# quantumjot/sequitr

Hardware: AMD Instinct MI355X
Metric: segmented Mpixels/sec on 512x512 tiles; IoU vs reference (higher is better)
Workload: dtype f32; 1 GPU; U-Net 2-class inference, launches of 32 512x512x1 tiles, fp32 (BASELINE.json configs[1]: filters 16-32-64-128-256, eltwise_mul bridge); logits + uint8 argmax mask; one 32-tile batch per GPU per step; tiles_this_rank=32

## Files before the change

### include/sequitr_hip.h

```cpp
#ifndef SEQUITR_HIP_H
#define SEQUITR_HIP_H

#include <stdint.h>

#ifdef __cplusplus
extern "C" {
#endif

#define SQ_OK 0
#define SQ_EINVAL (-1)
#define SQ_ELAUNCH (-2)
#define SQ_EALIGN (-3)

#define SQ_ACT_NONE 0
#define SQ_ACT_RELU 1
#define SQ_ACT_LEAKY 2

#define SQ_BRIDGE_NONE 0
#define SQ_BRIDGE_ADD 1
#define SQ_BRIDGE_MUL 2
#define SQ_BRIDGE_SUB 3

int sq_version(void);
const char *sq_last_error(void);
// ... 126 lines not shown
int sq_wgan_losses_fwd_f32(const float *Dz, const float *Dx, const float *gn2, float *out2, int N, void *stream);
int sq_wgan_losses_bwd_f32(const float *Dz, const float *Dx, const float *gn2, const float *g_dloss, const float *g_gloss,
                           float *dDz, float *dDx, float *dgn2, int N, void *stream);

int sq_mosaic_pack_f32(const float *x, float *m, int N, int H, int W, int C, int R, int Cc, void *stream);
int sq_mosaic_unpack_f32(const float *m, float *y, int N, int H, int W, int C, int R, int Cc, void *stream);

int64_t sq_dense_workspace_f32(int M, int K, int N);
int sq_dense_fwd_f32(const float *x, const float *w, const float *bias, float *y, float *workspace, int M, int K, int N,
                     float wscale, int act, void *stream);
int sq_dense_wgrad_f32(const float *x, const float *dy, float *dw, float *db, int M, int K, int N, float scale, int accumulate,
                       void *stream);

int64_t sq_wgrad1x1_small_workspace_f32(int64_t npix, int Ca, int Cb);
int sq_wgrad1x1_small_f32(const float *a, const float *b, float *m, float *workspace, int64_t npix, int Ca, int Cb,
                          void *stream);


int sq_conv2d_concat_nhwc_fwd_f32(const float *xa, const float *xb, const float *w, const float *bias, float *y, int N,
                                  int H, int W, int Ca, int Cout, int K, int act, void *stream);

int sq_conv3x3_pool_fwd_f32(const float *x, const float *w, const float *bias, float *y, float *pooled,
                            int N, int H, int W, int Cin, int Cout, int act, void *stream);

int sq_conv3x3_head_fwd_f32(const float *x, const float *w, const float *bias, const float *head_w,
                            const float *head_b, float *logits, uint8_t *mask, int N, int H, int W,
                            int Cin, int head_c, int act, void *stream);

int sq_conv3x3_first_block_fwd_f32(const float *x, const float *w1, const float *b1, const float *w2,
                                   const float *b2, float *y, float *pooled, int N, int H, int W,
                                   void *stream);

int sq_convT_conv3x3_fwd_f32(const float *x_low, const float *wt, const float *bt, const float *skip, int bridge,
                             const float *w, const float *bias, float *y, int N, int H, int W, int act, void *stream);


int64_t sq_conv_packed_weights_elems_bf16(int K, int Cin, int Cout);
int sq_conv_pack_weights_bf16(const float *w, void *wp, int K, int Cin, int Cout, float wscale, int transform,
                              void *stream);
int sq_conv_pack_weights_multi_bf16(const float *base, void *out, const int32_t *table, int n_entries,
                                    int total_items, void *stream);
int sq_conv_pack_weights_multi_scaled_bf16(const float *base, void *out, const int32_t *table, const float *scales,
                                           int n_entries, int total_items, void *stream);

int sq_conv2d_nhwc_fwd_bf16(const void *x, const void *wp, const float *bias, void *y, int N, int H, int W,
                            int Cin, int Cout, int K, int act, void *stream);
// ... 423 lines not shown
```

### sequitr_amd/_lib.py

```python
import ctypes
import os

_HERE = os.path.dirname(os.path.abspath(__file__))
LIB_PATH = os.path.join(_HERE, "_build", "libsequitr_hip.so")

c_void_p, c_int, c_float, c_int64 = ctypes.c_void_p, ctypes.c_int, ctypes.c_float, ctypes.c_int64


class WgradItem(ctypes.Structure):
    _fields_ = [("x", c_void_p), ("dy", c_void_p), ("dw", c_void_p), ("db", c_void_p),
                ("N", ctypes.c_int32), ("H", ctypes.c_int32), ("W", ctypes.c_int32), ("Cin", ctypes.c_int32),
                ("Cout", ctypes.c_int32), ("K", ctypes.c_int32), ("convT_cout", ctypes.c_int32), ("dw_scale", c_float),
                ("accumulate", ctypes.c_int32), ("mosaic_R", ctypes.c_int32), ("mosaic_Cc", ctypes.c_int32),
                ("reserved", ctypes.c_int32)]

SIGNATURES = {
    "sq_version": (c_int, []),
    "sq_last_error": (ctypes.c_char_p, []),
    "sq_conv2d_nhwc_fwd_f32": (c_int, [c_void_p] * 4 + [c_int] * 6 + [c_float, c_int, c_void_p]),
    "sq_maxpool2x2_fwd_f32": (c_int, [c_void_p] * 2 + [c_int] * 4 + [c_void_p]),
    "sq_avgpool2x2_fwd_f32": (c_int, [c_void_p] * 2 + [c_int] * 4 + [c_void_p]),
    "sq_convT2x2s2_nhwc_fwd_f32": (c_int, [c_void_p] * 5 + [c_int] * 6 + [c_void_p]),
    "sq_bridge_fwd_f32": (c_int, [c_void_p] * 3 + [c_int64, c_int, c_void_p]),
    "sq_conv1x1_argmax_fwd_f32": (c_int, [c_void_p] * 5 + [c_int] * 5 + [c_void_p]),
# ... 127 lines not shown
    "sq_broadcast2x2_act_bwd_f32": (c_int, [c_void_p] * 3 + [c_int] * 4 + [c_float, c_int, c_void_p]),
    "sq_resize_nearest_f32": (c_int, [c_void_p] * 2 + [c_int] * 6 + [c_void_p]),
    "sq_lerp_f32": (c_int, [c_void_p] * 3 + [c_int64, c_int64, c_float, c_void_p, c_void_p]),
    "sq_scale_f32": (c_int, [c_void_p] * 2 + [c_int64, c_int64, c_float, c_void_p, c_int, c_void_p]),
    "sq_act_fwd_f32": (c_int, [c_void_p] * 2 + [c_int64, c_int, c_void_p]),
    "sq_dot_per_sample_workspace_f32": (c_int64, [c_int]),
    "sq_dot_per_sample_f32": (c_int, [c_void_p] * 4 + [c_int, c_int64, c_void_p]),
    "sq_mbstd_fwd_f32": (c_int, [c_void_p] * 3 + [c_int, c_int64, c_void_p]),
    "sq_mbstd_map_workspace": (c_int64, [c_int]),
    "sq_mbstd_map_fwd_f32": (c_int, [c_void_p] * 3 + [c_int, c_int, c_int64, c_int, c_void_p]),
    "sq_mbstd_map_bwd_f32": (c_int, [c_void_p] * 4 + [c_int, c_int, c_int64, c_int, c_void_p]),
    "sq_mbstd_map_bwd2_f32": (c_int, [c_void_p] * 6 + [c_int, c_int, c_int64, c_int, c_void_p]),
    "sq_mbstd_map_fwd_bf16": (c_int, [c_void_p] * 3 + [c_int, c_int, c_int64, c_int, c_void_p]),
    "sq_mbstd_map_bwd_bf16": (c_int, [c_void_p] * 4 + [c_int, c_int, c_int64, c_int, c_void_p]),
    "sq_mbstd_map_bwd2_bf16": (c_int, [c_void_p] * 6 + [c_int, c_int, c_int64, c_int, c_void_p]),
    "sq_wgan_losses_fwd_f32": (c_int, [c_void_p] * 4 + [c_int, c_void_p]),
    "sq_wgan_losses_bwd_f32": (c_int, [c_void_p] * 8 + [c_int, c_void_p]),
    "sq_dense_wgrad_f32": (c_int, [c_void_p] * 4 + [c_int] * 3 + [c_float, c_int, c_void_p]),
    "sq_wgrad1x1_small_workspace_f32": (c_int64, [c_int64, c_int, c_int]),
    "sq_wgrad1x1_small_f32": (c_int, [c_void_p] * 4 + [c_int64, c_int, c_int, c_void_p]),
    "sq_conv2d_concat_nhwc_fwd_f32": (c_int, [c_void_p] * 5 + [c_int] * 7 + [c_void_p]),
    "sq_conv3x3_pool_fwd_f32": (c_int, [c_void_p] * 5 + [c_int] * 6 + [c_void_p]),
    "sq_conv3x3_head_fwd_f32": (c_int, [c_void_p] * 7 + [c_int] * 6 + [c_void_p]),
    "sq_conv3x3_first_block_fwd_f32": (c_int, [c_void_p] * 7 + [c_int] * 3 + [c_void_p]),
    "sq_conv_packed_weights_elems_bf16": (c_int64, [c_int] * 3),
    "sq_conv_pack_weights_bf16": (c_int, [c_void_p] * 2 + [c_int] * 3 + [c_float, c_int, c_void_p]),
    "sq_conv2d_nhwc_fwd_bf16": (c_int, [c_void_p] * 4 + [c_int] * 7 + [c_void_p]),
    "sq_conv2d_nhwc_fwd_mixed_f32": (c_int, [c_void_p] * 4 + [c_int] * 7 + [c_void_p]),
    "sq_conv2d_nhwc_wgrad_workspace_mixed_f32": (c_int64, [c_int] * 6),
    "sq_conv2d_nhwc_wgrad_mixed_f32": (c_int, [c_void_p] * 5 + [c_int] * 6 + [c_void_p]),
    "sq_conv2d_nhwc_wgrad_scaled_mixed_f32": (c_int, [c_void_p] * 5 + [c_int] * 6 + [c_float, c_void_p]),
    "sq_conv2d_nhwc_wgrad_scaled_f32": (c_int, [c_void_p] * 5 + [c_int] * 6 + [c_float, c_void_p]),
    "sq_conv3x3_first_fwd_bf16": (c_int, [c_void_p] * 4 + [c_int] * 6 + [c_void_p]),
    "sq_conv2d_nhwc_wgrad_workspace_bf16": (c_int64, [c_int] * 6),
    "sq_conv2d_nhwc_wgrad_bf16": (c_int, [c_void_p] * 5 + [c_int] * 6 + [c_void_p]),
    "sq_convT2x2s2_wgrad_bf16": (c_int, [c_void_p] * 5 + [c_int] * 5 + [c_void_p]),
    "sq_cast_f32_to_bf16": (c_int, [c_void_p] * 2 + [c_int64, c_void_p]),
    "sq_cast_bf16_to_f32": (c_int, [c_void_p] * 2 + [c_int64, c_void_p]),
    "sq_head_concat_fwd_bf16": (c_int, [c_void_p] * 3 + [c_int64, c_int, c_void_p]),
    "sq_head_concat_bwd_bf16": (c_int, [c_void_p] * 3 + [c_int64, c_int, c_void_p]),
    "sq_maxpool2x2_fwd_bf16": (c_int, [c_void_p] * 2 + [c_int] * 4 + [c_void_p]),
    "sq_maxpool2x2_bwd_bf16": (c_int, [c_void_p] * 3 + [c_int] * 4 + [c_void_p]),
    "sq_conv_pack_weights_multi_bf16": (c_int, [c_void_p, c_void_p, c_void_p, c_int, c_int, c_void_p]),
    "sq_conv_pack_weights_multi_scaled_bf16": (c_int, [c_void_p] * 4 + [c_int, c_int, c_void_p]),
    "sq_conv2d_nhwc_fwd_dropout_bf16": (c_int, [c_void_p] * 4 + [c_int] * 7 + [c_float, ctypes.c_uint32, c_void_p, c_void_p]),
    "sq_conv3x3_first_fwd_mask_bf16": (c_int, [c_void_p] * 5 + [c_int] * 6 + [c_void_p]),
# ... 99 lines not shown
```

### sequitr_amd/networks/unet.py

```python
import contextlib
import logging

import numpy as np
import torch

from .. import functional as F
from .. import functional_bf16 as FB
from .. import ops

DEFAULT_FILTERS = (16, 32, 64, 128, 256)
DEFAULT_DROPOUT = 0.4
BRIDGE_TYPES = ('eltwise_add', 'eltwise_mul', 'eltwise_sub', 'concat', None)

TRAIN, EVAL, PREDICT = 'train', 'eval', 'infer'

logger = logging.getLogger('worker_process')


def variance_scaling(shape, rng, scale=1.0):
    fan_in = float(shape[-2] * int(np.prod(shape[:-2])))
    std = np.sqrt(scale / max(1.0, fan_in)) / .87962566103423978
    out = rng.standard_normal(size=shape)
    bad = np.abs(out) > 2.0
    while bad.any():
# ... 191 lines not shown
        dev = params.get('device', None)
        self.device = torch.device(dev) if dev is not None else torch.device('cuda', torch.cuda.current_device())
        if self.device.type != 'cuda':
            raise RuntimeError('UNet2D runs on the HIP back end only (device=%s)' % self.device)
        if tuple(self.kernel) not in ((3, 3), (1, 1)):
            raise ValueError('kernel %s unsupported: the HIP conv kernels are 3x3 or 1x1' % (self.kernel,))
        self._params = dict(params)
        self._seed = params.get('seed', 0)
        self._rng = np.random.default_rng(self._seed)
        self._vars = {}
        self._loaded, self._creatable = False, set()
        self._dropout_calls = 0
        self._builds = 0
        self.dropout_masks = None
        self.fuse = bool(params.get('fuse', True))
        self.fuse_up = bool(params.get('fuse_up', True))
        self.up_kernel = tuple(params.get('up_kernel', (2, 2)))
        if self.up_kernel not in ((2, 2), (3, 3)):
            raise ValueError('up_kernel %s unsupported: (2,2) or (3,3)' % (self.up_kernel,))
        self.batch_norm = bool(params.get('batch_norm', False))
        self.bn_eps = float(params.get('bn_epsilon', ops.BN_EPS))
        self.bn_momentum = float(params.get('bn_momentum', ops.BN_MOMENTUM))
        self._mask = None

    @classmethod
    def variable_shapes(cls, params):
        return unet_variable_shapes(params)

    def get_variable(self, name, shape, init):
        key = self.scope + '/' + name
        v = self._vars.get(key)
        if v is None:
            if self._loaded and key not in self._creatable:
                raise KeyError('variable %s is not in the loaded model (load_state_dict(strict=False) to allow '
                               'missing variables to be initialised)' % key)
            v = torch.from_numpy(init(shape)).to(self.device)
            self._vars[key] = v
        elif tuple(v.shape) != tuple(shape):
            raise ValueError('variable %s has shape %s, wanted %s' % (key, tuple(v.shape), tuple(shape)))
        return v

    def _kernel(self, shape):
        return self.get_variable('kernel', shape, lambda s: variance_scaling(s, self._rng))

    def _bias(self, n):
        return self.get_variable('bias', (n,), lambda s: np.zeros(s, np.float32))
# ... 5 lines not shown
        req = dict(unet_variable_shapes(self._params))
        opt = {}
        if self.batch_norm:
            for k, shp in list(req.items()):
                if k.endswith('/gamma'):
                    sc = k.rsplit('/', 1)[0]
                    opt[sc + '/moving_mean'] = opt[sc + '/moving_variance'] = shp
        return req, opt

    def load_state_dict(self, weights, strict=True):
        req, opt = self.expected_variables()
        if strict:
            missing = [k for k in req if k not in weights]
            unexpected = [k for k in weights if k not in req and k not in opt]
            bad = [(k, tuple(np.shape(weights[k])), tuple(s)) for k, s in list(req.items()) + list(opt.items())
                   if k in weights and tuple(np.shape(weights[k])) != tuple(s)]
            if missing or unexpected or bad:
                raise ValueError('load_state_dict: model does not fit this %s configuration -- missing %s; unexpected %s; '
                                 'shape mismatches (key, got, wanted) %s' % (self.__class__.__name__, missing[:6],
                                                                             unexpected[:6], bad[:6]))
            self._loaded, self._creatable = True, set(opt)
        for k, v in weights.items():
            self._vars[k] = torch.as_tensor(np.ascontiguousarray(v, dtype=np.float32)).to(self.device)

    def initialize(self):
        self.load_state_dict(self._initial_weights(), strict=False)
        return self

    def _initial_weights(self):
        return init_unet_weights(self._params, self._seed)

    def reshape_input(self, features):
        if isinstance(features, np.ndarray):
            features = torch.from_numpy(np.require(features, np.float32, ['C', 'W']))
        if not isinstance(features, torch.Tensor):
            raise TypeError('features must be a numpy array or a torch tensor')
        features = features.to(self.device, dtype=torch.float32, non_blocking=True)
        return UNet.reshape_input(self, features).contiguous()

    def conv_layer(self, x, filters):
        k = tuple(self.kernel)
        w, b = self._kernel(k + (x.shape[-1], filters)), self._bias(filters)
        if self.batch_norm:
            z = F.conv2d(x, w, b, act=None) if self.training else ops.conv2d(x, w, b, act=None)
            return self.batch_norm_layer(z, act='relu')
        if self.training:
            return F.conv2d(x, w, b, act='relu')
        return ops.conv2d(x, w, b, act='relu')

    def batch_norm_layer(self, z, act=None):
        n = z.shape[-1]
        gamma = self.get_variable('gamma', (n,), lambda s: np.ones(s, np.float32))
        beta = self.get_variable('beta', (n,), lambda s: np.zeros(s, np.float32))
        mmean = self.get_variable('moving_mean', (n,), lambda s: np.zeros(s, np.float32))
        mvar = self.get_variable('moving_variance', (n,), lambda s: np.ones(s, np.float32))
        if self.training:
            return F.batch_norm_train(z, gamma, beta, mmean, mvar, self.bn_eps, self.bn_momentum, act=act)
        return ops.bn_inference(z, gamma, beta, mmean, mvar, self.bn_eps, act=act)

    def conv_layer_1x1(self, x, filters):
        w, b = self._kernel((1, 1, x.shape[-1], filters)), self._bias(filters)
        small = filters <= 7 and x.shape[-1] % 4 == 0
        if self.training:
            if small and filters <= 4 and x.shape[-1] in (8, 16, 32):
                return F.conv1x1_head(x, w, b)
            return F.conv2d(x, w, b, act=None)
        if small:
            logits, self._mask = ops.conv1x1_argmax(x, w, b)
            return logits
        return ops.conv2d(x, w, b, act=None)

# ... 77 lines not shown
    def _v(self, path, kind, shape):
        scopes = path.split('/')
        self._scopes.extend(scopes)
        try:
            return self._kernel(shape) if kind == 'kernel' else self._bias(shape[0])
        finally:
            del self._scopes[-len(scopes):]

    def _build_fused(self, features):
        f = list(self.filters)
        L = len(f)
        x = self.reshape_input(features)
        net, pooled = [], None
        for i in range(L):
            s = 'UNet/down%d' % i
            cin = x.shape[-1] if i == 0 else f[i - 1]
            w1, b1 = self._v(s + '/conv1', 'kernel', (3, 3, cin, f[i])), self._v(s + '/conv1', 'bias', (f[i],))
            w2, b2 = self._v(s + '/conv2', 'kernel', (3, 3, f[i], f[i])), self._v(s + '/conv2', 'bias', (f[i],))
            src = x if i == 0 else pooled
            last = i == L - 1
            if i == 0 and cin == 1 and f[0] == 16:
                y, pooled = ops.conv3x3_first_block(src, w1, b1, w2, b2, want_pool=not last)
            else:
                c1 = ops.conv2d(src, w1, b1, act='relu')
                if last:
                    y, pooled = ops.conv2d(c1, w2, b2, act='relu'), None
                else:
                    y, pooled = ops.conv3x3_pool(c1, w2, b2, act='relu')
            net.append(y)
        head_fused = f[0] == 16 and self.n_outputs <= 4
        logits = None
        for i in reversed(range(L - 1)):
            s = 'UNet/up%d' % i
            wt, bt = self._v(s + '/upscale', 'kernel', (2, 2, f[i], f[i + 1])), self._v(s + '/upscale', 'bias', (f[i],))
            w1, b1 = self._v(s + '/conv1', 'kernel', (3, 3, f[i], f[i])), self._v(s + '/conv1', 'bias', (f[i],))
            w2, b2 = self._v(s + '/conv2', 'kernel', (3, 3, f[i], f[i])), self._v(s + '/conv2', 'bias', (f[i],))
            if f[i] == 16 and f[i + 1] == 32 and self.fuse_up:
                c1 = ops.convT_conv3x3(net[-1], wt, bt, net[i], self.bridge_type, w1, b1, act='relu')
            else:
                merged = ops.convT2x2s2(net[-1], wt, bt, skip=net[i], bridge=self.bridge_type)
                c1 = ops.conv2d(merged, w1, b1, act='relu')
            if i == 0 and head_fused:
                wh = self._v('UNet/to_image', 'kernel', (1, 1, f[0], self.n_outputs))
                bh = self._v('UNet/to_image', 'bias', (self.n_outputs,))
                logits, self._mask = ops.conv3x3_head(c1, w2, b2, wh, bh, act='relu')
                net.append(None)
            else:
                net.append(ops.conv2d(c1, w2, b2, act='relu'))
        if logits is None:
            wh = self._v('UNet/to_image', 'kernel', (1, 1, f[0], self.n_outputs))
            bh = self._v('UNet/to_image', 'bias', (self.n_outputs,))
            if self.n_outputs <= 7:
                logits, self._mask = ops.conv1x1_argmax(net[-1], wh, bh)
            else:
                logits = ops.conv2d(net[-1], wh, bh, act=None)
        net.append(logits)
        self._net = net
        return logits

    def predict(self, features):
        logits = self.build(features)
        if self._mask is None or self._mask.shape != logits.shape[:-1]:
            self._mask = ops.argmax_u8(logits)
        return self._mask

    def predict_stream(self, tiles, batch=32, want_logits=False, pipe=None, on_batch=None):
        from ..frontend import segment_tiles
        return segment_tiles(self, tiles, batch=batch, want_logits=want_logits, pipe=pipe, on_batch=on_batch)


class UNet_LEGACY(UNet2D):
# ... 74 lines not shown
    def __init__(self, net, batch_shape, warmup=2):
        if net.training:
            raise RuntimeError('GraphedPredict captures the inference graph (mode infer / eval)')
        self.net = net
        self.x = torch.zeros(tuple(batch_shape), dtype=torch.float32, device=net.device)
        side = torch.cuda.Stream(device=net.device)
        side.wait_stream(torch.cuda.current_stream(net.device))
        with torch.cuda.stream(side):
            for _ in range(max(1, warmup)):
                net.predict(self.x)
        torch.cuda.current_stream(net.device).wait_stream(side)
        torch.cuda.synchronize(net.device)
        self.graph = torch.cuda.CUDAGraph()
        with torch.cuda.graph(self.graph):
            self.mask = net.predict(self.x)
            self.logits = net.logits()

    def __call__(self, features):
        if isinstance(features, np.ndarray):
            features = torch.from_numpy(np.require(features, np.float32, ['C', 'W']))
        if tuple(features.shape) != tuple(self.x.shape):
            raise ValueError('captured for %s, got %s' % (tuple(self.x.shape), tuple(features.shape)))
        self.x.copy_(features, non_blocking=True)
        self.graph.replay()
        return self.mask, self.logits


class UNet2DBf16(UNet2D):

    def __init__(self, params, mode=PREDICT):
        UNet2D.__init__(self, dict(params, fuse=False), mode)
        self.fuse_block = bool(params.get('fuse_block', True))
        self._skip_boxes = {}
        if not 1 <= self.n_inputs <= 7:
            raise ValueError('the bf16 graph takes an f32 image of 1..7 channels (num_inputs)')
        if any(f % 16 for f in self.filters) or self.bridge_type == 'concat':
            raise ValueError('the bf16 graph needs filter counts that are multiples of 16 and an eltwise bridge')
        k = self.bridge_type
        self.bridge = (lambda x, y, _k=k: FB.bridge(x, y, _k)) if k else (lambda x, y: x)
        self._default_bridge = self.bridge

    def conv_layer(self, x, filters):
        w, b = self._kernel((3, 3, x.shape[-1], filters)), self._bias(filters)
        act = None if self.batch_norm else 'relu'
        z = FB.conv3x3_first(x, w, b, act=act) if x.dtype == torch.float32 else FB.conv2d(x, w, b, act=act)
        return self.batch_norm_layer(z, act='relu') if self.batch_norm else z
# ... 265 lines not shown
```

### sequitr_amd/ops.py

```python
import os

import torch

from . import _lib

ACT = {None: 0, "none": 0, "relu": 1, "leaky": 2}
BRIDGE = {None: 0, "none": 0, "eltwise_add": 1, "eltwise_mul": 2, "eltwise_sub": 3}


def _stream():
    return torch.cuda.current_stream().cuda_stream


def _chk(t, name, dtype=torch.float32, ndim=None):
    if not isinstance(t, torch.Tensor):
        raise TypeError("%s must be a torch.Tensor" % name)
    if not t.is_cuda:
        raise _lib.SequitrHipError("%s must live in GPU memory (no CPU fallback exists)" % name)
    if t.dtype != dtype:
        raise TypeError("%s must be %s, got %s" % (name, dtype, t.dtype))
    if not t.is_contiguous():
        raise ValueError("%s must be contiguous (NHWC)" % name)
    if ndim is not None and t.dim() != ndim:
        raise ValueError("%s must have %d dims, got %s" % (name, ndim, tuple(t.shape)))
# ... 136 lines not shown
        self.scales = torch.tensor(scales if scales else [1.0], dtype=torch.float32, device=dev)
        self.out = torch.zeros(max(dst, 8), dtype=torch.bfloat16, device=dev)
        self.leaves = [entry[1] for entry in named]
        _PLANS.add(self)

    def run(self):
        if self.n:
            _lib.check(_lib.load().sq_conv_pack_weights_multi_scaled_bf16(
                _ptr(self.flat), _ptr(self.out), _ptr(self.table), _ptr(self.scales), self.n, self.total, _stream()),
                "sq_conv_pack_weights_multi_scaled_bf16")
        self.fresh = True

    def lookup(self, w, K, Cin, Cout, wscale, transform):
        base = w._base if w._base is not None else w
        e = self.views.get((id(base), bool(transform)))
        if e is None or not self.fresh:
            return None
        d0, n, ws, k, ci, co = e
        if (k, ci, co) != (K, Cin, Cout) or ws != float(wscale):
            return None
        return self.out[d0:d0 + n]


def _packed_filter(w, K, Cin, Cout, wscale, transform):
    for plan in list(_PLANS):
        wp = plan.lookup(w, K, Cin, Cout, wscale, transform)
        if wp is not None:
            return wp
    cacheable = w.is_leaf and w.requires_grad
    key = (w.data_ptr(), K, Cin, Cout, float(wscale), bool(transform))
    if cacheable and key in _PACKS:
        return _PACKS[key][1]
    lib = _lib.load()
    n = lib.sq_conv_packed_weights_elems_bf16(K, Cin, Cout)
    wp = torch.empty((n,), dtype=torch.bfloat16, device=w.device)
    _lib.check(lib.sq_conv_pack_weights_bf16(_ptr(w), _ptr(wp), K, Cin, Cout, float(wscale), 1 if transform else 0,
                                            _stream()), "sq_conv_pack_weights_bf16")
    if cacheable:
        _PACKS[key] = (w, wp)
    return wp


def _conv2d_mixed(x, w, bias, act, wscale, y, transform):
    N, H, W, Cin = x.shape
    K, Cout = w.shape[0], (w.shape[2] if transform else w.shape[3])
    lib = _lib.load()
# ... 14 lines not shown
    lib = _lib.load()
    ws = _workspace(lib.sq_dense_workspace_f32(M, K, N), x.device)
    y = torch.empty((M, N), dtype=torch.float32, device=x.device)
    _lib.check(lib.sq_dense_fwd_f32(_ptr(x), _ptr(w), _ptr(bias), _ptr(y), _ptr(ws), M, K, N, float(wscale), ACT[act],
                                   _stream()), "sq_dense_fwd_f32")
    return y


def dense_wgrad(x, dy, want_bias=True, dw_scale=1.0, shape4=False, dw_out=None, db_out=None, accumulate=0):
    _chk(x, "x", ndim=2), _chk(dy, "dy", ndim=2)
    M, K = x.shape
    N = dy.shape[1]
    if dy.shape[0] != M:
        raise ValueError("dense_wgrad: x %s and dy %s differ in rows" % (tuple(x.shape), tuple(dy.shape)))
    dw = _grad_out(dw_out, (K, N), x.device) if dw_out is not None else torch.empty(
        (1, 1, K, N) if shape4 else (K, N), dtype=torch.float32, device=x.device)
    db = (_grad_out(db_out, (N,), x.device) if db_out is not None else torch.empty((N,), dtype=torch.float32, device=x.device)) \
        if want_bias else None
    _lib.check(_lib.load().sq_dense_wgrad_f32(_ptr(x), _ptr(dy), _ptr(dw), _ptr(db), M, K, N, float(dw_scale), int(accumulate),
                                             _stream()), "sq_dense_wgrad_f32")
    return dw, db


def conv2d(x, w, bias=None, act=None, wscale=1.0, out=None, _dgrad=False):
    if out is None and (x.dtype == _BF16 or STORE_BF16) and _gb().takes(x, w, _dgrad):
        return _gb().conv2d(x, w, bias, act, wscale, _dgrad)
    _chk(x, "x", ndim=4), _chk(w, "w", ndim=4)
    N, H, W, Cin = x.shape
    if _dgrad:
        takes_dense = out is None and w.shape[0] == 1 and N * H * W <= 128 and Cin >= 1024 and Cin % 4 == 0 and USE_DENSE
        if takes_dense or not (MIXED and Cin % 8 == 0 and w.shape[2] % 4 == 0):
            w, _dgrad = conv_weight_transform(w), False
    K, K2, Ci, Cout = w.shape
    if _dgrad:
        Ci, Cout = Cout, Ci
    if K != K2 or Ci != Cin:
        raise ValueError("weight shape %s does not match input channels %d" % (tuple(w.shape), Cin))
    if bias is not None:
        _chk(bias, "bias")
        if bias.numel() != Cout:
            raise ValueError("bias must have %d elements" % Cout)
    if out is None and K == 1 and N * H * W <= 128 and Cin >= 1024 and Cin % 4 == 0 and USE_DENSE:
        return dense(x.view(N * H * W, Cin), w.view(Cin, Cout), bias, act, wscale).view(N, H, W, Cout)
    if out is None and USE_MOSAIC and W < 16 and N * H > 1:
        P = N * H * W
        if K == 1 and P % 16 == 0:
            return conv2d(x.view(1, P // 16, 16, Cin), w, bias, act, wscale, _dgrad=_dgrad).view(N, H, W, Cout)
        plan = _mosaic_plan(N, H, W) if (K == 3 and Cin % 4 == 0 and Cout % 4 == 0) else None
        if plan is not None and MOSAIC_IN_KERNEL and MIXED and Cin % 8 == 0:
            wp = _packed_filter(w, K, Cin, Cout, wscale, _dgrad)
            y = torch.empty((N, H, W, Cout), dtype=torch.float32, device=x.device)
            _lib.check(_lib.load().sq_conv2d_nhwc_mixed_mosaic_f32(_ptr(x), _ptr(wp), _ptr(bias), None, _ptr(y), N, H, W, Cin,
                                                                  Cout, ACT[act], plan[0], plan[1], _stream()),
                       "sq_conv2d_nhwc_mixed_mosaic_f32")
            return y
        if plan is not None:
            ym = conv2d(mosaic_pack(x, *plan), w, bias, act, wscale, _dgrad=_dgrad)
            return mosaic_unpack(ym, N, H, W, *plan)
    y = _out(out, (N, H, W, Cout), x)
    if MIXED and Cin % 8 == 0 and Cout % 4 == 0:
        return _conv2d_mixed(x, w, bias, act, wscale, y, _dgrad)
    lib = _lib.load()
    _lib.check(lib.sq_conv2d_nhwc_fwd_f32(_ptr(x), _ptr(w), _ptr(bias), _ptr(y), N, H, W, Cin, Cout, K,
                                         float(wscale), ACT[act], _stream()), "sq_conv2d_nhwc_fwd_f32")
    return y


def conv2d_concat(xa, xb, w, bias=None, act=None):
    _chk(xa, "xa", ndim=4), _chk(xb, "xb", ndim=4), _chk(w, "w", ndim=4)
    if tuple(xa.shape) != tuple(xb.shape):
        raise ValueError("conv2d_concat: the two sources differ in shape: %s vs %s" % (tuple(xa.shape), tuple(xb.shape)))
    N, H, W, Ca = xa.shape
    K, K2, Cin, Cout = w.shape
    if K != K2 or Cin != 2 * Ca:
        raise ValueError("conv2d_concat: weight %s does not match 2 x %d input channels" % (tuple(w.shape), Ca))
    if bias is not None:
        _chk(bias, "bias")
    y = torch.empty((N, H, W, Cout), dtype=torch.float32, device=xa.device)
    _lib.check(_lib.load().sq_conv2d_concat_nhwc_fwd_f32(_ptr(xa), _ptr(xb), _ptr(w), _ptr(bias), _ptr(y), N, H, W, Ca, Cout,
                                                        K, ACT[act], _stream()), "sq_conv2d_concat_nhwc_fwd_f32")
    return y


def _pool(x, fn_name, out):
    _chk(x, "x", ndim=4)
# ... 843 lines not shown
    lib = _lib.load()
    if Cout % 4 == 0 and lib.sq_conv2d_nhwc_wgrad_workspace_f32(N, H, W, Cin, Cout, K) >= 0:
        if Cin <= 7 and dw_scale != 1.0:
            dw, db = conv2d_wgrad(x, dy, K, want_bias=want_bias, dw_out=dw_out, db_out=db_out)
            return dw * dw_scale, db
        return conv2d_wgrad(x, dy, K, want_bias=want_bias, dw_out=dw_out, db_out=db_out, dw_scale=dw_scale)
    if dw_scale != 1.0:
        dw, db = conv_wgrad_raw(x, dy, K, want_bias=want_bias, dw_out=dw_out, db_out=db_out)
        return dw * dw_scale, db
    if dw_out is not None or db_out is not None:
        raise _lib.SequitrHipError("conv wgrad: gradient destinations need the MFMA kernel (Cin=%d Cout=%d)" % (Cin, Cout))
    npix = N * H * W
    if K == 1 and Cin <= 7 and Cout % 4 == 0:
        dw = wgrad1x1_small(x, dy).view(1, 1, Cin, Cout)
        db = wgrad1x1_small(_ones(npix, 1, x.device), dy).view(Cout) if want_bias else None
        return dw, db
    if K == 1 and Cout <= 7 and Cin % 4 == 0:
        dw = wgrad1x1_small(dy, x).t().contiguous().view(1, 1, Cin, Cout)
        db = wgrad1x1_small(dy, _ones(npix, 4, x.device))[:, 0].contiguous() if want_bias else None
        return dw, db
    raise _lib.SequitrHipError("conv wgrad: unsupported Cin=%d Cout=%d K=%d" % (Cin, Cout, K))


def conv3x3_pool(x, w, bias, act="relu"):
    _chk(x, "x", ndim=4), _chk(w, "w", ndim=4)
    N, H, W, Cin = x.shape
    Cout = w.shape[3]
    if tuple(w.shape[:3]) != (3, 3, Cin):
        raise ValueError("conv3x3_pool: weight %s does not match %d input channels" % (tuple(w.shape), Cin))
    if bias is not None:
        _chk(bias, "bias")
    y = torch.empty((N, H, W, Cout), dtype=torch.float32, device=x.device)
    p = torch.empty((N, H // 2, W // 2, Cout), dtype=torch.float32, device=x.device)
    lib = _lib.load()
    _lib.check(lib.sq_conv3x3_pool_fwd_f32(_ptr(x), _ptr(w), _ptr(bias), _ptr(y), _ptr(p), N, H, W, Cin, Cout,
                                          ACT[act], _stream()), "sq_conv3x3_pool_fwd_f32")
    return y, p


def conv3x3_head(x, w, bias, head_w, head_b, act="relu", want_mask=True):
    _chk(x, "x", ndim=4), _chk(w, "w", ndim=4), _chk(head_w, "head_w", ndim=4)
    N, H, W, Cin = x.shape
    if tuple(w.shape) != (3, 3, Cin, 16) or tuple(head_w.shape[:3]) != (1, 1, 16):
        raise ValueError("conv3x3_head needs w (3,3,%d,16) and head_w (1,1,16,C)" % Cin)
    hc = head_w.shape[3]
    logits = torch.empty((N, H, W, hc), dtype=torch.float32, device=x.device)
    mask = torch.empty((N, H, W), dtype=torch.uint8, device=x.device) if want_mask else None
    lib = _lib.load()
    _lib.check(lib.sq_conv3x3_head_fwd_f32(_ptr(x), _ptr(w), _ptr(bias), _ptr(head_w), _ptr(head_b), _ptr(logits),
                                          _ptr(mask), N, H, W, Cin, hc, ACT[act], _stream()), "sq_conv3x3_head_fwd_f32")
    return logits, mask


def convT_conv3x3(x_low, wt, bt, skip, bridge, w, bias, act="relu"):
    _chk(x_low, "x_low", ndim=4), _chk(wt, "wt", ndim=4), _chk(skip, "skip", ndim=4), _chk(w, "w", ndim=4)
    N, H, W, C = skip.shape
    if C != 16 or tuple(x_low.shape) != (N, H // 2, W // 2, 32) or tuple(wt.shape) != (2, 2, 16, 32) \
# ... 319 lines not shown
```

Before: 1650 Mpixels/s.

## Add prepacked f32 3x3 conv filters with a register-ring MFMA kernel

Adds a one-time kernel that repacks 3x3 f32 conv filters into per-lane float4 MFMA operand order, plus a new f32 MFMA conv kernel that streams those packed weights through a small register ring of buffer loads while double-buffering the input halo in LDS. The UNet inference path packs each eligible kernel when weights are loaded and passes the pack to conv2d and conv3x3_pool. Before each graph replay the packs are revalidated against an invalidation epoch. The aim is to cut weight-load address math and LDS traffic for weights in the wide layers, at the cost of extra device memory for the packs, a repack check on every replay, and fallbacks when shapes or the plan's block width do not qualify.

Result: faster. 1686 Mpixels/s, median of 6 (+2.2%).

```diff
diff --git a/include/sequitr_hip.h b/include/sequitr_hip.h
--- a/include/sequitr_hip.h
+++ b/include/sequitr_hip.h
@@ -172,6 +172,14 @@
 
 int sq_conv3x3_pool_fwd_f32(const float *x, const float *w, const float *bias, float *y, float *pooled,
                             int N, int H, int W, int Cin, int Cout, int act, void *stream);
+
+int64_t sq_conv_packed_filter_elems_f32(int K, int Cin, int Cout);
+int sq_conv_pack_filter_f32(const float *w, float *wp, int K, int Cin, int Cout, void *stream);
+int sq_conv_packed_takes_f32(int N, int H, int W, int Cin, int Cout, int K);
+int sq_conv2d_packed_nhwc_fwd_f32(const float *x, const float *w, const float *wp, const float *bias, float *y, int N, int H,
+                                  int W, int Cin, int Cout, int K, float wscale, int act, void *stream);
+int sq_conv3x3_pool_packed_fwd_f32(const float *x, const float *w, const float *wp, const float *bias, float *y, float *pooled,
+                                   int N, int H, int W, int Cin, int Cout, int act, void *stream);
 
 int sq_conv3x3_head_fwd_f32(const float *x, const float *w, const float *bias, const float *head_w,
                             const float *head_b, float *logits, uint8_t *mask, int N, int H, int W,
diff --git a/sequitr_amd/_lib.py b/sequitr_amd/_lib.py
--- a/sequitr_amd/_lib.py
+++ b/sequitr_amd/_lib.py
@@ -173,6 +173,11 @@
     "sq_conv2d_concat_nhwc_fwd_f32": (c_int, [c_void_p] * 5 + [c_int] * 7 + [c_void_p]),
     "sq_conv3x3_pool_fwd_f32": (c_int, [c_void_p] * 5 + [c_int] * 6 + [c_void_p]),
     "sq_conv3x3_head_fwd_f32": (c_int, [c_void_p] * 7 + [c_int] * 6 + [c_void_p]),
+    "sq_conv_packed_filter_elems_f32": (c_int64, [c_int] * 3),
+    "sq_conv_pack_filter_f32": (c_int, [c_void_p] * 2 + [c_int] * 3 + [c_void_p]),
+    "sq_conv_packed_takes_f32": (c_int, [c_int] * 6),
+    "sq_conv2d_packed_nhwc_fwd_f32": (c_int, [c_void_p] * 5 + [c_int] * 6 + [c_float, c_int, c_void_p]),
+    "sq_conv3x3_pool_packed_fwd_f32": (c_int, [c_void_p] * 6 + [c_int] * 6 + [c_void_p]),
     "sq_conv3x3_first_block_fwd_f32": (c_int, [c_void_p] * 7 + [c_int] * 3 + [c_void_p]),
     "sq_conv_packed_weights_elems_bf16": (c_int64, [c_int] * 3),
     "sq_conv_pack_weights_bf16": (c_int, [c_void_p] * 2 + [c_int] * 3 + [c_float, c_int, c_void_p]),
diff --git a/sequitr_amd/csrc/sq_conv_f32_packed.hip b/sequitr_amd/csrc/sq_conv_f32_packed.hip
--- /dev/null
+++ b/sequitr_amd/csrc/sq_conv_f32_packed.hip
@@ -0,0 +1,331 @@
+#include <stdlib.h>
+#include <type_traits>
+#include "sq_common.h"
+#include "sq_conv_epi.h"
+
+#ifndef SQ_PK_RING
+#define SQ_PK_RING 4
+#endif
+#ifndef SQ_PK_OCC
+#define SQ_PK_OCC 2
+#endif
+#ifndef SQ_PK_WRITE_AT
+#define SQ_PK_WRITE_AT 22
+#endif
+
+namespace {
+
+constexpr int TH = 16, TW = 16, BN = 64, KC = 16, NR = BN / 16;
+constexpr int HALO_W = TW + 2, HALO_H = TH + 2, HP = HALO_W * HALO_H;
+constexpr int PS = KC + 2;
+constexpr int XS_FLOATS = HP * PS;
+constexpr int QPP = KC / 4, XITEMS = HP * QPP, XSLOTS = (XITEMS + 255) / 256;
+constexpr int NSTEP = 9 * (KC / 4);
+constexpr int RING = SQ_PK_RING;
+constexpr int STEP_BYTES = 64 * 16, ITEM_BYTES = NSTEP * STEP_BYTES;
+constexpr int LDS_BYTES = (2 * XS_FLOATS + 64 * 4) * 4;
+constexpr int OCC = SQ_PK_OCC;
+static_assert(SQ_PK_OCC != 2 || sq_v2_occ(BN, KC, false) == 2, "the default walks the unpacked form's grid");
+static_assert(NSTEP % RING == 0 && RING >= 2 && RING <= 6, "the ring slot of a step must not depend on the item");
+static_assert(SQ_PK_WRITE_AT + XSLOTS <= NSTEP, "the halo writes must fit the item's steps");
+static_assert((XS_FLOATS * 4) % 16 == 0, "second halo buffer must start 16-B aligned");
+
+__global__ __launch_bounds__(256) void pack_filter_f32_kernel(const float *__restrict__ w, float4 *__restrict__ wp,
+                                                              int Cin, int Cout, int total) {
+    const int e = blockIdx.x * 256 + threadIdx.x;
+    if (e >= total) return;
+    const int lane = e & 63, li = lane & 15, kk = lane >> 4;
+    int t = e >> 6;
+    const int s = t & 3;
+    t >>= 2;
+    const int tap = t % 9;
+    t /= 9;
+    const int nchunk = Cin / KC, c = t % nchunk, cb = t / nchunk;
+    const float *src = w + (size_t)(tap * Cin + c * KC + 4 * s + kk) * Cout + cb * BN + li;
+    wp[e] = make_float4(src[0], src[16], src[32], src[48]);
+}
+
+__global__ __launch_bounds__(256, OCC) void conv_mfma_f32_packed_kernel(
+    const float *__restrict__ x, const float *__restrict__ wp, const float *__restrict__ bias, float *__restrict__ y,
+    int N, int H, int W, int Cin, int Cout, int act, int tiles_x, int tiles_y, int ntiles, float *__restrict__ pooled) {
+    extern __shared__ __attribute__((aligned(16))) float smem[];
+    const int tid = threadIdx.x, lane = tid & 63, wv = tid >> 6;
+    __builtin_assume(tid < 256);
+    const int li = lane & 15, kk = lane >> 4;
+    const int n0 = blockIdx.y * BN;
+    const int vb = (int)sq_xcd_remap(blockIdx.x, gridDim.x);
+    const int tstride = (int)gridDim.x;
+    const int t_begin = vb;
+    if (t_begin >= ntiles) return;
+    const int t_count = (ntiles - vb + tstride - 1) / tstride;
+    const int nchunk = Cin / KC;
+    const int nitems = t_count * nchunk;
+
+    const __amdgpu_buffer_rsrc_t xrsrc = __builtin_amdgcn_make_buffer_rsrc(
+        const_cast<float *>(x), 0, (int)((size_t)N * H * W * Cin * 4), 0x00020000);
+    const __amdgpu_buffer_rsrc_t wrsrc = __builtin_amdgcn_make_buffer_rsrc(
+        const_cast<float *>(wp), 0, 9 * Cin * Cout * 4, 0x00020000);
+    const __amdgpu_buffer_rsrc_t yrsrc = __builtin_amdgcn_make_buffer_rsrc(y, 0, (int)((size_t)N * H * W * Cout * 4), 0x00020000);
+    constexpr unsigned OOB = 0x80000000u;
+
+    int xrel[XSLOTS], xpy[XSLOTS], xpx[XSLOTS];
+#pragma unroll
+    for (int sl = 0; sl < XSLOTS; ++sl) {
+        const int idx = tid + sl * 256;
+        const int pix = idx / QPP, q = idx % QPP;
+        xpy[sl] = idx < XITEMS ? pix / HALO_W : (1 << 24);
+        xpx[sl] = pix % HALO_W;
+        xrel[sl] = idx < XITEMS ? ((pix / HALO_W * W + xpx[sl]) * Cin + q * 4) * 4 : (int)OOB;
+    }
+    float4 xr[XSLOTS];
+    auto issue = [&](int tx, int ty, int n, int cc, bool live) {
+        const int x0 = tx * TW - 1, y0 = ty * TH - 1;
+        const int base = (((n * H + y0) * W + x0) * Cin + cc) * 4;
+        const unsigned Hl = live ? (unsigned)H : 0u;
+#pragma unroll
+        for (int sl = 0; sl < XSLOTS; ++sl) {
+            const bool inb = (unsigned)(y0 + xpy[sl]) < Hl && (unsigned)(x0 + xpx[sl]) < (unsigned)W;
+            const unsigned off = inb ? (unsigned)(base + xrel[sl]) : OOB;
+            const auto v = __builtin_amdgcn_raw_buffer_load_b128(xrsrc, off, 0, 0);
+            xr[sl] = *reinterpret_cast<const float4 *>(&v);
+        }
+    };
+    float *const dump = smem + 2 * XS_FLOATS + lane * 4;
+    auto put_slot = [&](float *xs, int sl) {
+        const int idx = tid + sl * 256;
+        const int pix = idx / QPP, q = idx % QPP;
+        float *d = idx < XITEMS ? xs + pix * PS + q * 4 : dump;
+        *reinterpret_cast<float2 *>(d) = make_float2(xr[sl].x, xr[sl].y);
+        *reinterpret_cast<float2 *>(d + 2) = make_float2(xr[sl].z, xr[sl].w);
+    };
+
+    const int a_lane = lane * 16;
+    auto load_a = [&](int item_off, int st) {
+        const auto v = __builtin_amdgcn_raw_buffer_load_b128(wrsrc, a_lane, item_off + st * STEP_BYTES, 0);
+        return *reinterpret_cast<const float4 *>(&v);
+    };
+    const int xb_off = ((4 * wv) * HALO_W + li) * PS + kk;
+    auto load_b = [&](const float *xs, int st, float (&b)[4]) {
+        const int tap = st / 4, s = st % 4;
+        const int ky = tap / 3, kx = tap % 3;
+#pragma unroll
+        for (int r = 0; r < 4; ++r) b[r] = xs[xb_off + ((r + ky) * HALO_W + kx) * PS + s * 4];
+    };
+
+    const float slope = act == SQ_ACT_LEAKY ? 0.2f : 1.0f;
+    const bool is_relu = act == SQ_ACT_RELU;
+    auto actk = [&](float v, auto fastc) {
+        if constexpr (decltype(fastc)::value) return __builtin_fmaxf(v, 0.0f);
+        else {
+            const float neg = is_relu ? 0.0f : v * slope;
+            return v > 0.0f ? v : neg;
+        }
+    };
+    float4 bvr[NR];
+#pragma unroll
+    for (int nb = 0; nb < NR; ++nb)
+        bvr[nb] = bias ? *reinterpret_cast<const float4 *>(bias + n0 + nb * 16 + 4 * kk) : make_float4(0.f, 0.f, 0.f, 0.f);
+    const int fast_lane = (((4 * wv) * W + li) * Cout + 4 * kk) * 4;
+
+    f32x4 acc[4][NR];
+    auto epilogue = [&](int tx, int ty, int n, auto fastc) {
+        constexpr bool FAST = decltype(fastc)::value;
+        auto actf = [&](float v) { return actk(v, fastc); };
+        const int gx = tx * TW + li;
+#pragma unroll
+        for (int nb = 0; nb < NR; ++nb) {
+            const int co = n0 + nb * 16 + 4 * kk;
+            const float4 bv = bvr[nb];
+            f32x4 o[4];
+#pragma unroll
+            for (int r = 0; r < 4; ++r) {
+                const int gy = ty * TH + 4 * wv + r;
+                o[r][0] = actf(bias ? acc[r][nb][0] + bv.x : acc[r][nb][0]);
+                o[r][1] = actf(bias ? acc[r][nb][1] + bv.y : acc[r][nb][1]);
+                o[r][2] = actf(bias ? acc[r][nb][2] + bv.z : acc[r][nb][2]);
+                o[r][3] = actf(bias ? acc[r][nb][3] + bv.w : acc[r][nb][3]);
+                unsigned off;
+                if constexpr (FAST) {
+                    off = (unsigned)(fast_lane + nb * 64) + (unsigned)((((n * H + ty * TH + r) * W + tx * TW) * Cout + n0) * 4);
+                } else {
+                    const bool ok = gy < H && gx < W;
+                    off = ok ? (unsigned)((((n * H + gy) * W + gx) * Cout + co) * 4) : OOB;
+                }
+                __builtin_amdgcn_raw_buffer_store_b128(
+                    *reinterpret_cast<__attribute__((__vector_size__(4 * sizeof(unsigned)))) unsigned *>(&o[r]), yrsrc, off, 0, 0);
+                acc[r][nb] = (f32x4){0.f, 0.f, 0.f, 0.f};
+            }
+            if (pooled) {
+#pragma unroll
+                for (int pr = 0; pr < 2; ++pr) {
+                    float mp[4];
+#pragma unroll
+                    for (int j = 0; j < 4; ++j) {
+                        const float a = o[2 * pr][j], b = o[2 * pr + 1][j];
+                        const float v = b > a ? b : a;
+                        const float u = __shfl_xor(v, 1);
+                        mp[j] = u > v ? u : v;
+                    }
+                    const int py = (ty * TH + 4 * wv) / 2 + pr, px = gx >> 1;
+                    if ((li & 1) == 0 && py < (H >> 1) && px < (W >> 1))
+                        *reinterpret_cast<float4 *>(pooled + ((size_t)(n * (H >> 1) + py) * (W >> 1) + px) * Cout + co) =
+                            make_float4(mp[0], mp[1], mp[2], mp[3]);
+                }
+            }
+        }
+    };
+
+    const int per_image = tiles_x * tiles_y;
+    const int s_n = tstride / per_image, s_y = (tstride % per_image) / tiles_x, s_x = (tstride % per_image) % tiles_x;
+    int ctx = t_begin % tiles_x, cty = (t_begin / tiles_x) % tiles_y, cn = t_begin / per_image;
+    int ntx = ctx + s_x, nty = cty, nn = cn;
+    if (ntx >= tiles_x) { ntx -= tiles_x; nty += 1; }
+    nty += s_y;
+    if (nty >= tiles_y) { nty -= tiles_y; nn += 1; }
+    nn += s_n;
+
+    const int cb_off = blockIdx.y * nchunk * ITEM_BYTES;
+    issue(ctx, cty, cn, 0, true);
+    float4 ar[RING];
+#pragma unroll
+    for (int j = 0; j < RING; ++j) ar[j] = load_a(cb_off, j);
+#pragma unroll
+    for (int sl = 0; sl < XSLOTS; ++sl) put_slot(smem, sl);
+#pragma unroll
+    for (int r = 0; r < 4; ++r)
+#pragma unroll
+        for (int nb = 0; nb < NR; ++nb) acc[r][nb] = (f32x4){0.f, 0.f, 0.f, 0.f};
+    __syncthreads();
+
+    int chunk = 0;
+    for (int it = 0; it < nitems; ++it) {
+        const float *xs = smem + (it & 1) * XS_FLOATS;
+        float *xo = smem + ((it & 1) ^ 1) * XS_FLOATS;
+        int nchk = chunk + 1;
+        const bool same = nchk != nchunk;
+        if (!same) nchk = 0;
+        const bool has_next = it + 1 < nitems;
+        issue(same ? ctx : ntx, same ? cty : nty, same ? cn : nn, nchk * KC, has_next);
+        const int item_off = cb_off + chunk * ITEM_BYTES, next_off = cb_off + nchk * ITEM_BYTES;
+        {
+            float b0[4], b1[4];
+            load_b(xs, 0, b0);
+            __builtin_amdgcn_s_setprio(0);
+#pragma unroll
+            for (int st = 0; st < NSTEP; ++st) {
+                float (&bc)[4] = (st & 1) ? b1 : b0;
+                float (&bn)[4] = (st & 1) ? b0 : b1;
+                const float4 a = ar[st % RING];
+                if (st + 1 < NSTEP) load_b(xs, st + 1, bn);
+                if (st >= SQ_PK_WRITE_AT && st < SQ_PK_WRITE_AT + XSLOTS) put_slot(xo, st - SQ_PK_WRITE_AT);
+                __builtin_amdgcn_sched_barrier(0);
+                const float av[NR] = {a.x, a.y, a.z, a.w};
+#pragma unroll
+                for (int r = 0; r < 4; ++r)
+#pragma unroll
+                    for (int nb = 0; nb < NR; ++nb)
+                        acc[r][nb] = __builtin_amdgcn_mfma_f32_16x16x4f32(av[nb], bc[r], acc[r][nb], 0, 0, 0);
+                ar[st % RING] = st + RING < NSTEP ? load_a(item_off, st + RING) : load_a(next_off, st + RING - NSTEP);
+                __builtin_amdgcn_sched_barrier(0);
+            }
+            __builtin_amdgcn_s_setprio(3);
+        }
+        __syncthreads();
+        if (!same) {
+            const bool fast = is_relu && cty * TH + TH <= H && ctx * TW + TW <= W;
+            if (fast) epilogue(ctx, cty, cn, std::integral_constant<bool, true>{});
+            else epilogue(ctx, cty, cn, std::integral_constant<bool, false>{});
+            ctx = ntx; cty = nty; cn = nn;
+            ntx += s_x;
+            if (ntx >= tiles_x) { ntx -= tiles_x; nty += 1; }
+            nty += s_y;
+            if (nty >= tiles_y) { nty -= tiles_y; nn += 1; }
+            nn += s_n;
+        }
+        chunk = nchk;
+    }
+}
+
+bool packed_switch_on() {
+    const char *e = getenv("SQ_CONV_PACKED");
+    return !(e && e[0] == '0');
+}
+
+bool pack_eligible(int K, int Cin, int Cout) { return K == 3 && Cin > 0 && Cin % KC == 0 && Cout > 0 && Cout % BN == 0; }
+
+}
+
+extern "C" int64_t sq_conv_packed_filter_elems_f32(int K, int Cin, int Cout) {
+    return pack_eligible(K, Cin, Cout) ? (int64_t)9 * Cin * Cout : -1;
+}
+
+extern "C" int sq_conv_pack_filter_f32(const float *w, float *wp, int K, int Cin, int Cout, void *stream) {
+    SQ_REQUIRE(w && wp, "sq_conv_pack_filter_f32: null pointer");
+    SQ_REQUIRE(pack_eligible(K, Cin, Cout), "sq_conv_pack_filter_f32: unsupported K=%d Cin=%d Cout=%d (3x3, Cin %% 16 == 0, Cout %% 64 == 0)",
+               K, Cin, Cout);
+    SQ_REQUIRE((int64_t)9 * Cin * Cout * 4 < ((int64_t)1 << 31), "sq_conv_pack_filter_f32: the pack must be < 2 GiB");
+    SQ_REQUIRE_ALIGNED(w); SQ_REQUIRE_ALIGNED(wp);
+    const int total = 9 * Cin * Cout / 4;
+    hipLaunchKernelGGL(pack_filter_f32_kernel, dim3((total + 255) / 256), dim3(256), 0, reinterpret_cast<hipStream_t>(stream),
+                       w, reinterpret_cast<float4 *>(wp), Cin, Cout, total);
+    return sq_check_launch("sq_conv_pack_filter_f32");
+}
+
+extern "C" int sq_conv_packed_takes_f32(int N, int H, int W, int Cin, int Cout, int K) {
+    if (N <= 0 || H <= 0 || W <= 0 || !pack_eligible(K, Cin, Cout) || !packed_switch_on()) return 0;
+    if ((size_t)N * H * W * (size_t)(Cin > Cout ? Cin : Cout) * 4 >= ((size_t)1 << 31)) return 0;
+    const int64_t ntiles = (int64_t)((W + TW - 1) / TW) * ((H + TH - 1) / TH) * N;
+    return sq_plan_f32_bn(ntiles, Cout) == 64 ? 1 : 0;
+}
+
+static int sq_conv_packed_launch(const float *x, const float *wp, const float *bias, float *y, float *pooled, int N, int H, int W,
+                          int Cin, int Cout, int act, hipStream_t st) {
+    static bool attr_set = false;
+    if (!attr_set) {
+        if (hipFuncSetAttribute(reinterpret_cast<const void *>(conv_mfma_f32_packed_kernel),
+                                hipFuncAttributeMaxDynamicSharedMemorySize, LDS_BYTES) != hipSuccess) {
+            sq_set_error("conv_mfma_f32_packed: cannot reserve %d bytes of LDS", LDS_BYTES);
+            return SQ_ELAUNCH;
+        }
+        attr_set = true;
+    }
+    const int tiles_x = (W + TW - 1) / TW, tiles_y = (H + TH - 1) / TH;
+    const int ntiles = tiles_x * tiles_y * N;
+    const int gy = Cout / BN;
+    int tpb;
+    const int gx = sq_plan_v2_grid(ntiles, gy, OCC, &tpb);
+    hipLaunchKernelGGL(conv_mfma_f32_packed_kernel, dim3(gx, gy), dim3(256), LDS_BYTES, st, x, wp, bias, y, N, H, W, Cin, Cout,
+                       act, tiles_x, tiles_y, ntiles, pooled);
+    return sq_check_launch("sq_conv2d_packed_nhwc_fwd_f32");
+}
+
+namespace {
+int packed_args_ok(const char *who, const float *x, const float *wp, const float *bias, const float *y, const float *pooled,
+                   int N, int H, int W, int Cin, int Cout, int act) {
+    SQ_REQUIRE(x && y, "%s: null tensor pointer", who);
+    SQ_REQUIRE(act >= SQ_ACT_NONE && act <= SQ_ACT_LEAKY, "%s: bad activation %d", who, act);
+    SQ_REQUIRE_ALIGNED(x); SQ_REQUIRE_ALIGNED(wp); SQ_REQUIRE_ALIGNED(y);
+    if (bias) SQ_REQUIRE_ALIGNED(bias);
+    if (pooled) SQ_REQUIRE_ALIGNED(pooled);
+    return SQ_OK;
+}
+}
+
+extern "C" int sq_conv2d_packed_nhwc_fwd_f32(const float *x, const float *w, const float *wp, const float *bias, float *y,
+                                             int N, int H, int W, int Cin, int Cout, int K, float wscale, int act, void *stream) {
+    static const bool impl1 = [] { const char *e = getenv("SQ_CONV_IMPL"); return e && e[0] == '1'; }();
+    if (!wp || wscale != 1.0f || impl1 || !sq_conv_packed_takes_f32(N, H, W, Cin, Cout, K))
+        return sq_conv2d_nhwc_fwd_f32(x, w, bias, y, N, H, W, Cin, Cout, K, wscale, act, stream);
+    const int rc = packed_args_ok("sq_conv2d_packed_nhwc_fwd_f32", x, wp, bias, y, nullptr, N, H, W, Cin, Cout, act);
+    if (rc != SQ_OK) return rc;
+    return sq_conv_packed_launch(x, wp, bias, y, nullptr, N, H, W, Cin, Cout, act, reinterpret_cast<hipStream_t>(stream));
+}
+
+extern "C" int sq_conv3x3_pool_packed_fwd_f32(const float *x, const float *w, const float *wp, const float *bias, float *y,
+                                              float *pooled, int N, int H, int W, int Cin, int Cout, int act, void *stream) {
+    if (!wp || !pooled || H % 2 || W % 2 || !sq_conv_packed_takes_f32(N, H, W, Cin, Cout, 3))
+        return sq_conv3x3_pool_fwd_f32(x, w, bias, y, pooled, N, H, W, Cin, Cout, act, stream);
+    const int rc = packed_args_ok("sq_conv3x3_pool_packed_fwd_f32", x, wp, bias, y, pooled, N, H, W, Cin, Cout, act);
+    if (rc != SQ_OK) return rc;
+    return sq_conv_packed_launch(x, wp, bias, y, pooled, N, H, W, Cin, Cout, act, reinterpret_cast<hipStream_t>(stream));
+}
diff --git a/sequitr_amd/networks/unet.py b/sequitr_amd/networks/unet.py
--- a/sequitr_amd/networks/unet.py
+++ b/sequitr_amd/networks/unet.py
@@ -237,6 +237,7 @@
         self.bn_eps = float(params.get('bn_epsilon', ops.BN_EPS))
         self.bn_momentum = float(params.get('bn_momentum', ops.BN_MOMENTUM))
         self._mask = None
+        self._packs = {}
 
     @classmethod
     def variable_shapes(cls, params):
@@ -288,6 +289,22 @@
             self._loaded, self._creatable = True, set(opt)
         for k, v in weights.items():
             self._vars[k] = torch.as_tensor(np.ascontiguousarray(v, dtype=np.float32)).to(self.device)
+        self._packs = {}
+        if not self.training and not self.batch_norm and type(self).conv_layer is UNet2D.conv_layer:
+            for k in weights:
+                if k.endswith('/kernel'):
+                    self._wpack(k, self._vars[k])
+
+    def _wpack(self, key, w):
+        e = self._packs.get(key, False)
+        if e is False or (e is not None and e.w is not w):
+            e = self._packs[key] = ops.pack_filter(w)
+        return e
+
+    def refresh_packs(self):
+        for e in self._packs.values():
+            if e is not None:
+                e.current(e.w)
 
     def initialize(self):
         self.load_state_dict(self._initial_weights(), strict=False)
@@ -312,7 +329,7 @@
             return self.batch_norm_layer(z, act='relu')
         if self.training:
             return F.conv2d(x, w, b, act='relu')
-        return ops.conv2d(x, w, b, act='relu')
+        return ops.conv2d(x, w, b, act='relu', pack=self._wpack(self.scope + '/kernel', w))
 
     def batch_norm_layer(self, z, act=None):
         n = z.shape[-1]
@@ -436,11 +453,12 @@
             if i == 0 and cin == 1 and f[0] == 16:
                 y, pooled = ops.conv3x3_first_block(src, w1, b1, w2, b2, want_pool=not last)
             else:
-                c1 = ops.conv2d(src, w1, b1, act='relu')
+                p1, p2 = self._wpack(s + '/conv1/kernel', w1), self._wpack(s + '/conv2/kernel', w2)
+                c1 = ops.conv2d(src, w1, b1, act='relu', pack=p1)
                 if last:
-                    y, pooled = ops.conv2d(c1, w2, b2, act='relu'), None
+                    y, pooled = ops.conv2d(c1, w2, b2, act='relu', pack=p2), None
                 else:
-                    y, pooled = ops.conv3x3_pool(c1, w2, b2, act='relu')
+                    y, pooled = ops.conv3x3_pool(c1, w2, b2, act='relu', pack=p2)
             net.append(y)
         head_fused = f[0] == 16 and self.n_outputs <= 4
         logits = None
@@ -453,14 +471,14 @@
                 c1 = ops.convT_conv3x3(net[-1], wt, bt, net[i], self.bridge_type, w1, b1, act='relu')
             else:
                 merged = ops.convT2x2s2(net[-1], wt, bt, skip=net[i], bridge=self.bridge_type)
-                c1 = ops.conv2d(merged, w1, b1, act='relu')
+                c1 = ops.conv2d(merged, w1, b1, act='relu', pack=self._wpack(s + '/conv1/kernel', w1))
             if i == 0 and head_fused:
                 wh = self._v('UNet/to_image', 'kernel', (1, 1, f[0], self.n_outputs))
                 bh = self._v('UNet/to_image', 'bias', (self.n_outputs,))
                 logits, self._mask = ops.conv3x3_head(c1, w2, b2, wh, bh, act='relu')
                 net.append(None)
             else:
-                net.append(ops.conv2d(c1, w2, b2, act='relu'))
+                net.append(ops.conv2d(c1, w2, b2, act='relu', pack=self._wpack(s + '/conv2/kernel', w2)))
         if logits is None:
             wh = self._v('UNet/to_image', 'kernel', (1, 1, f[0], self.n_outputs))
             bh = self._v('UNet/to_image', 'bias', (self.n_outputs,))
@@ -581,6 +599,7 @@
         if tuple(features.shape) != tuple(self.x.shape):
             raise ValueError('captured for %s, got %s' % (tuple(self.x.shape), tuple(features.shape)))
         self.x.copy_(features, non_blocking=True)
+        self.net.refresh_packs()
         self.graph.replay()
         return self.mask, self.logits
 
diff --git a/sequitr_amd/ops.py b/sequitr_amd/ops.py
--- a/sequitr_amd/ops.py
+++ b/sequitr_amd/ops.py
@@ -182,6 +182,46 @@
         return self.out[d0:d0 + n]
 
 
+class FilterPackF32(object):
+
+    def __init__(self, w):
+        _chk(w, "w", ndim=4)
+        K, K2, Cin, Cout = w.shape
+        n = _lib.load().sq_conv_packed_filter_elems_f32(K, Cin, Cout) if K == K2 else -1
+        if n <= 0:
+            raise ValueError("no f32 filter pack for a %s filter (3x3, Cin %% 16 == 0, Cout %% 64 == 0)" % (tuple(w.shape),))
+        self.w = w
+        self.wp = torch.empty((n,), dtype=torch.float32, device=w.device)
+        self.epoch = None
+        self.repack()
+
+    def repack(self):
+        K, _, Cin, Cout = self.w.shape
+        self.epoch = invalidation_epoch()
+        _lib.check(_lib.load().sq_conv_pack_filter_f32(_ptr(self.w), _ptr(self.wp), K, Cin, Cout, _stream()),
+                   "sq_conv_pack_filter_f32")
+
+    def current(self, w):
+        if w is not self.w:
+            raise ValueError("pack= belongs to another filter tensor than the call's w")
+        if self.epoch != invalidation_epoch():
+            self.repack()
+        return self.wp
+
+
+def pack_filter(w):
+    if w.dim() != 4 or w.shape[0] != w.shape[1] or w.dtype != torch.float32:
+        return None
+    if _lib.load().sq_conv_packed_filter_elems_f32(w.shape[0], w.shape[2], w.shape[3]) <= 0:
+        return None
+    return FilterPackF32(w)
+
+
+def conv_packed_takes(x_shape, w_shape):
+    N, H, W, Cin = x_shape
+    return bool(_lib.load().sq_conv_packed_takes_f32(N, H, W, Cin, w_shape[3], w_shape[0])) and w_shape[2] == Cin
+
+
 def _packed_filter(w, K, Cin, Cout, wscale, transform):
     for plan in list(_PLANS):
         wp = plan.lookup(w, K, Cin, Cout, wscale, transform)
@@ -242,7 +282,7 @@
     return dw, db
 
 
-def conv2d(x, w, bias=None, act=None, wscale=1.0, out=None, _dgrad=False):
+def conv2d(x, w, bias=None, act=None, wscale=1.0, out=None, _dgrad=False, pack=None):
     if out is None and (x.dtype == _BF16 or STORE_BF16) and _gb().takes(x, w, _dgrad):
         return _gb().conv2d(x, w, bias, act, wscale, _dgrad)
     _chk(x, "x", ndim=4), _chk(w, "w", ndim=4)
@@ -281,6 +321,11 @@
     if MIXED and Cin % 8 == 0 and Cout % 4 == 0:
         return _conv2d_mixed(x, w, bias, act, wscale, y, _dgrad)
     lib = _lib.load()
+    if pack is not None and not _dgrad:
+        _lib.check(lib.sq_conv2d_packed_nhwc_fwd_f32(_ptr(x), _ptr(w), _ptr(pack.current(w)), _ptr(bias), _ptr(y), N, H, W, Cin,
+                                                    Cout, K, float(wscale), ACT[act], _stream()),
+                   "sq_conv2d_packed_nhwc_fwd_f32")
+        return y
     _lib.check(lib.sq_conv2d_nhwc_fwd_f32(_ptr(x), _ptr(w), _ptr(bias), _ptr(y), N, H, W, Cin, Cout, K,
                                          float(wscale), ACT[act], _stream()), "sq_conv2d_nhwc_fwd_f32")
     return y
@@ -1170,7 +1215,7 @@
     raise _lib.SequitrHipError("conv wgrad: unsupported Cin=%d Cout=%d K=%d" % (Cin, Cout, K))
 
 
-def conv3x3_pool(x, w, bias, act="relu"):
+def conv3x3_pool(x, w, bias, act="relu", pack=None):
     _chk(x, "x", ndim=4), _chk(w, "w", ndim=4)
     N, H, W, Cin = x.shape
     Cout = w.shape[3]
@@ -1181,6 +1226,10 @@
     y = torch.empty((N, H, W, Cout), dtype=torch.float32, device=x.device)
     p = torch.empty((N, H // 2, W // 2, Cout), dtype=torch.float32, device=x.device)
     lib = _lib.load()
+    if pack is not None:
+        _lib.check(lib.sq_conv3x3_pool_packed_fwd_f32(_ptr(x), _ptr(w), _ptr(pack.current(w)), _ptr(bias), _ptr(y), _ptr(p), N, H,
+                                                     W, Cin, Cout, ACT[act], _stream()), "sq_conv3x3_pool_packed_fwd_f32")
+        return y, p
     _lib.check(lib.sq_conv3x3_pool_fwd_f32(_ptr(x), _ptr(w), _ptr(bias), _ptr(y), _ptr(p), N, H, W, Cin, Cout,
                                           ACT[act], _stream()), "sq_conv3x3_pool_fwd_f32")
     return y, p
```
